# srv/pcl_feature_extraction

Hardware: AMD Instinct MI355X
Metric: Mpoints/s through NARF keypoint + FPFH descriptor on 1M-pt cloud (higher is better)
Workload: dtype f32; 1 GPU; configs[2] 1M-pt synthetic room, NARF(support 0.2) + normals(r 0.05) + FPFH(r 0.08) at the keypoints; image=640x480, parallelism=scan-per-gpu x1, descriptor_rows=83

## Files before the change

pcl_feature_extraction_amd/csrc/pfx_fpfh.hip:

```cpp
#include <cstring>
#include <rocprim/rocprim.hpp>

#include "pfx_nblist.h"
#include "pfx_neighbors.h"
#include "pfx_pair_features.h"

namespace pfx {
namespace {

constexpr int kBins = 11;
constexpr int kDesc = 33;
constexpr int kCapW = 8192;
constexpr int64_t kCapWGlobal = 1 << 22;
constexpr int kWOvfBlocks = 16;
constexpr int kChunkW = 128;
constexpr int kWT = 1024;
constexpr int kHistCopies = 16;


__device__ __forceinline__ bool bin_fast_nb(float v, float tol, int& h) {
  const float m = floorf(v);
  const float fr = v - m;
  h = (int)fminf(fmaxf(m, 0.0f), (float)(kBins - 1));
  return (fr > tol) & (fr < 1.0f - tol);
}

typedef float fv2 __attribute__((ext_vector_type(2)));
struct v32 { fv2 x, y, z; };
__device__ __forceinline__ fv2 dot4v(const v32& a, const v32& b) { return (a.x * b.x + a.z * b.z) + (a.y * b.y + 0.0f); }
__device__ __forceinline__ v32 cross3v(const v32& a, const v32& b) {
  return v32{a.y * b.z - a.z * b.y, a.z * b.x - a.x * b.z, a.x * b.y - a.y * b.x};
}
__device__ __forceinline__ fv2 sel2(bool c0, bool c1, fv2 a, fv2 b) { return fv2{c0 ? a.x : b.x, c1 ? a.y : b.y}; }

__device__ __forceinline__ void pair_bins_fast2(f3 p1, f3 n1, bool n1fin, const v32& p2, const v32& n2, int h1[2],
                                                int h2[2], int h3[2], bool ok[2]) {
  const int bz1 = bin_of<kBins>(f1_scaled<kBins>(0.0)), bz = bin_of<kBins>((double)kBins * ((0.0 + 1.0) * 0.5));
  const v32 dp0{p2.x - p1.x, p2.y - p1.y, p2.z - p1.z};
  const fv2 s4 = (dp0.x * dp0.x + dp0.z * dp0.z) + (dp0.y * dp0.y + 0.0f);
  const v32 n1v{fv2(n1.x), fv2(n1.y), fv2(n1.z)};
  const fv2 d1 = dot4v(n1v, dp0), d2 = dot4v(n2, dp0);
  bool sw[2], live[2];
  fv2 rf4;
#pragma unroll
  for (int c = 0; c < 2; ++c) {
    const bool fin = n1fin && isfinite(n2.x[c]) && isfinite(n2.y[c]) && isfinite(n2.z[c]);
    const float ad1 = fabsf(d1[c]), ad2 = fabsf(d2[c]);
    rf4[c] = __builtin_amdgcn_rsqf(s4[c]);
    sw[c] = ad1 < ad2 * (1.0f - 4e-7f);
    const bool decided = sw[c] || ad1 > ad2 * (1.0f + 4e-7f);
    live[c] = fin && !(fmaxf(ad1, ad2) * rf4[c] < 2e-8f) && decided;
  }
  const fv2 f3a = sel2(sw[0], sw[1], -d2 * rf4, d1 * rf4);
  const v32 n1c{sel2(sw[0], sw[1], n2.x, n1v.x), sel2(sw[0], sw[1], n2.y, n1v.y), sel2(sw[0], sw[1], n2.z, n1v.z)};
  const v32 n2c{sel2(sw[0], sw[1], n1v.x, n2.x), sel2(sw[0], sw[1], n1v.y, n2.y), sel2(sw[0], sw[1], n1v.z, n2.z)};
  const v32 dp{sel2(sw[0], sw[1], -dp0.x, dp0.x), sel2(sw[0], sw[1], -dp0.y, dp0.y), sel2(sw[0], sw[1], -dp0.z, dp0.z)};
  const v32 v = cross3v(dp, n1c);
  const fv2 sv = (v.x * v.x + v.z * v.z) + (v.y * v.y + 0.0f);
  const fv2 rsv{__builtin_amdgcn_rsqf(sv.x), __builtin_amdgcn_rsqf(sv.y)};
  const v32 vh{v.x * rsv, v.y * rsv, v.z * rsv};
  const v32 w = cross3v(n1c, vh);
  const fv2 f2a = dot4v(vh, n2c), y = dot4v(w, n2c), x = dot4v(n1c, n2c);
  fv2 mn, rmx;
  bool big[2];
#pragma unroll
  for (int c = 0; c < 2; ++c) {
    const float ax = fabsf(x[c]), ay = fabsf(y[c]);
    const float mx = fmaxf(ax, ay);
    mn[c] = fminf(ax, ay);
    big[c] = mx > 1e-20f;
    rmx[c] = __builtin_amdgcn_rcpf(mx);
  }
  const fv2 a = mn * rmx;
  const fv2 z = a * a;
  fv2 pp = fv2(-0.00405456405133009f);
  pp = pp * z + 0.021862948313355446f;
  pp = pp * z + -0.0559123195707798f;
  pp = pp * z + 0.0964219719171524f;
  pp = pp * z + -0.1390862911939621f;
  pp = pp * z + 0.19946566224098206f;
  pp = pp * z + -0.33329859375953674f;
  pp = pp * z + 0.9999993443489075f;
  fv2 t = pp * a;
#pragma unroll
  for (int c = 0; c < 2; ++c) {
    float tc = t[c];
    if (fabsf(y[c]) > fabsf(x[c])) tc = 1.57079637f - tc;
    if (x[c] < 0.0f) tc = 3.14159274f - tc;
    t[c] = y[c] < 0.0f ? -tc : tc;
  }
  const float d_pi = 1.0f / (2.0f * 3.14159265358979323846f);
  const fv2 tol1 = (fv2(1e-6f) + 8e-6f * rmx) * (1.01f * (float)kBins * d_pi) + kBinMapSlack;
  const fv2 b1 = (t + 3.14159265358979323846f) * ((float)kBins * d_pi);
  const fv2 b2 = (f2a + 1.0f) * (0.5f * kBins), b3 = (f3a + 1.0f) * (0.5f * kBins);
#pragma unroll
  for (int c = 0; c < 2; ++c) {
    int a1, a2, a3;
    const bool k1 = bin_fast_nb(b1[c], tol1[c], a1);
    const bool k2 = bin_fast_nb(b2[c], 4e-6f * 0.5f * kBins + kBinMapSlack, a2);
    const bool k3 = bin_fast_nb(b3[c], 1e-6f * 0.5f * kBins + kBinMapSlack, a3);
    const bool zero = s4[c] == 0.0f;
    ok[c] = zero | (live[c] & big[c] & k1 & k2 & k3);
    h1[c] = zero ? bz1 : a1;
    h2[c] = zero ? bz : a2;
    h3[c] = zero ? bz : a3;
  }
}

__device__ __attribute__((noinline)) int pair_bins_exact(float p1x, float p1y, float p1z, float n1x, float n1y,
                                                         float n1z, float p2x, float p2y, float p2z, float n2x,
                                                         float n2y, float n2z) {
  int h1, h2, h3;
  pair_bins<kBins>(mk3(p1x, p1y, p1z), mk3(n1x, n1y, n1z), mk3(p2x, p2y, p2z), mk3(n2x, n2y, n2z), h1, h2, h3);
  return h1 | (h2 << 8) | (h3 << 16);
}

__global__ void k_sorted_normals(const int32_t* __restrict__ perm, int64_t n, const float* __restrict__ nx,
                                 const float* __restrict__ ny, const float* __restrict__ nz,
                                 const uint8_t* __restrict__ support, float4* __restrict__ out,
                                 int* __restrict__ zero9) {
  const int64_t i = blockIdx.x * (int64_t)blockDim.x + threadIdx.x;
  if (zero9 && i < 9) zero9[i] = 0;
  if (i >= n) return;
  const int32_t p = perm[i];
  if (support && !support[p]) {
    out[i] = make_float4(__builtin_nanf(""), __builtin_nanf(""), __builtin_nanf(""), 0.0f);
    return;
  }
  out[i] = make_float4(nx[p], ny[p], nz[p], 0.0f);
}

__global__ void __launch_bounds__(256) k_fpfh_mark(GridView g, const float* __restrict__ qx,
                                                   const float* __restrict__ qy, const float* __restrict__ qz,
                                                   int64_t nq, float rr, uint8_t* __restrict__ flags) {
  for (int64_t q = blockIdx.x; q < nq; q += gridDim.x) {
    Runs R;
    const float x = qx[q], y = qy[q], z = qz[q];
    query_runs(g, x, y, z, R);
    for (int32_t t = threadIdx.x; t < R.pref[9]; t += blockDim.x) {
      const int32_t p = run_pos(R, t);
      const float4 c = g.sp[p];
      if (flann_d2(x, y, z, c.x, c.y, c.z) < rr) flags[p] = 1;
    }
  }
}

__global__ void __launch_bounds__(256) k_fpfh_mark_support(GridView g, const int32_t* __restrict__ plist,
                                                           const int64_t* __restrict__ n_ptr, float rr,
                                                           uint8_t* __restrict__ mask) {
  const int64_t n = *n_ptr;
  for (int64_t w = blockIdx.x; w < n; w += gridDim.x) {
    Runs R;
    const float4 q = g.sp[plist[w]];
    query_runs(g, q.x, q.y, q.z, R);
    for (int32_t t = threadIdx.x; t < R.pref[9]; t += blockDim.x) {
      const int32_t p = run_pos(R, t);
      const float4 c = g.sp[p];
      if (flann_d2(q.x, q.y, q.z, c.x, c.y, c.z) < rr) mask[g.perm[p]] = 1;
    }
  }
}

__global__ void __launch_bounds__(256) k_fpfh_mark_ball(GridView g, const float* __restrict__ qx,
                                                        const float* __restrict__ qy, const float* __restrict__ qz,
                                                        int64_t nq, float rr4, uint8_t* __restrict__ mask) {
  for (int64_t q = blockIdx.x; q < nq; q += gridDim.x) {
    const float x = qx[q], y = qy[q], z = qz[q];
    if (!(isfinite(x) && isfinite(y) && isfinite(z))) continue;
    const int64_t cx = (int64_t)floor(((double)x - g.ox) * g.inv);
    const int64_t cy = (int64_t)floor(((double)y - g.oy) * g.inv);
    const int64_t cz = (int64_t)floor(((double)z - g.oz) * g.inv);
    const int64_t z0 = max<int64_t>(cz - 2, 0), z1 = min<int64_t>(cz + 2, g.nz - 1);
    if (z0 > z1) continue;
    for (int c = 0; c < 25; ++c) {
      const int64_t ix = cx + c / 5 - 2, iy = cy + c % 5 - 2;
      if (ix < 0 || ix >= g.nx || iy < 0 || iy >= g.ny) continue;
      const int64_t base = (ix * g.ny + iy) * g.nz;
      const int32_t p0 = g.cell_start[base + z0], p1 = g.cell_start[base + z1 + 1];
      for (int32_t p = p0 + threadIdx.x; p < p1; p += blockDim.x) {
        const float4 c4 = g.sp[p];
        if (flann_d2(x, y, z, c4.x, c4.y, c4.z) <= rr4) mask[g.perm[p]] = 1;
      }
    }
  }
}

__global__ void k_all_finite(const uint32_t* __restrict__ skeys, int64_t n, uint64_t ncells,
                             uint8_t* __restrict__ flags) {
  const int64_t i = blockIdx.x * (int64_t)blockDim.x + threadIdx.x;
  if (i < n) flags[i] = (uint64_t)skeys[i] < ncells;
}

#ifndef PFX_SPFH_WPE
#define PFX_SPFH_WPE 7
#endif
__global__ void __launch_bounds__(256, PFX_SPFH_WPE) k_fpfh_spfh(GridView g, const float4* __restrict__ snp,
                                                      const int32_t* __restrict__ slist,
                                                      const int64_t* __restrict__ count_ptr, float rr,
                                                      int* __restrict__ hcount, int* __restrict__ kcount,
                                                      int2* __restrict__ slowq, unsigned* __restrict__ n_slow,
                                                      unsigned slow_cap, unsigned long long* __restrict__ pairs) {
  __shared__ uint32_t queue[4][192];
  __shared__ int hist[4][kHistCopies][kDesc];
  const int lane = threadIdx.x & 63, wv = __builtin_amdgcn_readfirstlane(threadIdx.x >> 6);
  const int64_t count = *count_ptr;
  const int64_t stride = (int64_t)gridDim.x * 4;
  unsigned long long wpairs = 0;
  for (int64_t w = xcd_block(blockIdx.x, gridDim.x) * 4 + wv; w < count; w += stride) {
    const int32_t s = __builtin_amdgcn_readfirstlane(slist[w]);
    float4 pc = g.sp[s], pnc = snp[s];
    pc.x = uniformf(pc.x); pc.y = uniformf(pc.y); pc.z = uniformf(pc.z);
    pnc.x = uniformf(pnc.x); pnc.y = uniformf(pnc.y); pnc.z = uniformf(pnc.z);
// ... 67 lines not shown
      for (int32_t t0 = 0; t0 < rn; t0 += 64) {
        const int32_t t = t0 + lane;
        bool hit = false;
        const int32_t pos = rs + t;
        if (t < rn) {
          const float4 c = g.sp[pos];
          hit = flann_d2(pc.x, pc.y, pc.z, c.x, c.y, c.z) < rr;
        }
        k += __popcll(__ballot(hit));
        const bool push = hit && pos != s;
        const uint64_t m = __ballot(push);
        if (push) queue[wv][qn + __popcll(m & lanemask_lt())] = (uint32_t)pos;
        qn += __popcll(m);
        if (qn >= 128) {
          process(128);
          const uint32_t rest = (lane + 128 < qn) ? queue[wv][lane + 128] : 0u;
          __builtin_amdgcn_fence(__ATOMIC_SEQ_CST, "wavefront");
          __builtin_amdgcn_wave_barrier();
          if (lane + 128 < qn) queue[wv][lane] = rest;
          qn -= 128;
        }
      }
    }
    process(qn);
    if (lane < kDesc) {
      int c = 0;
      for (int j = 0; j < kHistCopies; ++j) c += hist[wv][j][lane];
      hcount[w * kDesc + lane] = c;
    }
    if (lane == 0) kcount[w] = k;
    wpairs += (unsigned long long)(k - 1);
    __builtin_amdgcn_fence(__ATOMIC_SEQ_CST, "wavefront");
    __builtin_amdgcn_wave_barrier();
  }
  if (lane == 0 && wpairs) atomicAdd(pairs, wpairs);
}

__global__ void __launch_bounds__(256) k_fpfh_exact(GridView g, const float4* __restrict__ snp,
                                                    const int32_t* __restrict__ slist,
                                                    const int2* __restrict__ slowq, const unsigned* __restrict__ n_slow,
                                                    unsigned slow_cap, int* __restrict__ hcount,
                                                    unsigned long long* __restrict__ pairs) {
  const unsigned n = min(*n_slow, slow_cap);
  const unsigned i = blockIdx.x * 256 + threadIdx.x;
  if (i == 0) atomicAdd(pairs + 1, (unsigned long long)n);
  for (unsigned j = i; j < n; j += gridDim.x * 256) {
    const int2 e = slowq[j];
    const int32_t s = slist[e.x];
    const float4 pc = g.sp[s], pnc = snp[s], qc = g.sp[e.y], qnv = snp[e.y];
    const int hb = pair_bins_exact(pc.x, pc.y, pc.z, pnc.x, pnc.y, pnc.z, qc.x, qc.y, qc.z, qnv.x, qnv.y, qnv.z);
    int* hc = hcount + (int64_t)e.x * kDesc;
    atomicAdd(&hc[hb & 0xff], 1);
    atomicAdd(&hc[kBins + ((hb >> 8) & 0xff)], 1);
    atomicAdd(&hc[2 * kBins + (hb >> 16)], 1);
  }
}

__global__ void __launch_bounds__(256) k_fpfh_finalize(GridView g, const int32_t* __restrict__ slist,
                                                       const int64_t* __restrict__ count_ptr,
                                                       const int* __restrict__ hcount,
                                                       const int* __restrict__ kcount, float* __restrict__ spfh) {
  const int64_t count = *count_ptr;
  for (int64_t e = (int64_t)blockIdx.x * 256 + threadIdx.x; e < count * kDesc; e += (int64_t)gridDim.x * 256) {
    const int64_t w = e / kDesc;
    const int b = (int)(e - w * kDesc);
    const float incr = 100.0f / (float)(kcount[w] - 1);
    spfh[(int64_t)g.perm[slist[w]] * kDesc + b] = repeated_add(incr, hcount[e]);
  }
}

__device__ __forceinline__ int lsb_exp(float v) {
  const uint32_t b = __float_as_uint(v);
  const int e = (int)((b >> 23) & 0xff);
  if (e == 255) return 1000;
  const uint32_t m = (b & 0x7fffffu) | (e ? 0x800000u : 0u);
  return (e ? e : 1) - 150 + __builtin_ctz(m);
}

__device__ __forceinline__ int lsb_exp_bound(float v) {
  const int e = (int)((__float_as_uint(v) >> 23) & 0xff);
  return e == 255 ? 1000 : (e ? e : 1) - 150;
}

template <bool GLOBAL>
__global__ void __launch_bounds__(kWT) k_fpfh_weight(GridView g, const float* __restrict__ qx,
                                                     const float* __restrict__ qy, const float* __restrict__ qz,
                                                     int64_t nq, float rr, const float* __restrict__ spfh,
                                                     float* __restrict__ out, int* __restrict__ err,
                                                     int32_t* __restrict__ ovf, int* __restrict__ n_ovf,
                                                     uint64_t* __restrict__ scratch, int gcap) {
  extern __shared__ __attribute__((aligned(16))) uint64_t keys_lds[];
  __shared__ BucketLdsT<kWT> SB;
  uint64_t* keys = GLOBAL ? scratch + (size_t)blockIdx.x * gcap : keys_lds;
  const int kcap = GLOBAL ? gcap : kCapW;
  __shared__ float rows[kChunkW][kDesc + 1];
  __shared__ float wts[kChunkW];
  __shared__ double red_s[3][kWT / 64];
  __shared__ int red_l[3][kWT / 64];
  __shared__ int s_count;
  __shared__ double s_sum[3];
  const int tid = threadIdx.x;
  const int64_t count = GLOBAL ? (int64_t)*n_ovf : nq;
  for (int64_t w = blockIdx.x; w < count; w += gridDim.x) {
    const int64_t q = GLOBAL ? (int64_t)ovf[w] : w;
    const int k = GLOBAL ? sorted_neighbors(g, qx[q], qy[q], qz[q], rr, keys, kcap, &s_count)
                         : sorted_neighbors_bucketed<kWT>(g, qx[q], qy[q], qz[q], rr, keys, keys + kCapW, kcap,
                                                          &s_count, SB);
    if (k > kcap) {
      const bool give_up = GLOBAL || !ovf;
      if (tid == 0) {
        if (give_up) atomicMax(err, k);
        else ovf[atomicAdd(n_ovf, 1)] = (int32_t)q;
      }
      if (give_up && tid < kDesc) out[q * kDesc + tid] = __builtin_nanf("");
      continue;
    }
    if (k == 0) {
      if (tid < kDesc) out[q * kDesc + tid] = __builtin_nanf("");
      __syncthreads();
      continue;
    }
    float fh = 0.0f;
    double ps0 = 0.0, ps1 = 0.0, ps2 = 0.0;
    int pl0 = 1 << 20, pl1 = 1 << 20, pl2 = 1 << 20;
    constexpr int RS = kDesc + 1;
    float* rb0 = GLOBAL ? &rows[0][0] : reinterpret_cast<float*>(keys_lds + kCapW);
    float* rb1 = GLOBAL ? rb0 : rb0 + kChunkW * RS;
    const int nch = (k + kChunkW - 1) / kChunkW;
    auto stage = [&](int c, float* rbuf, int t0, int nt) {
      const int c0 = c * kChunkW, m = min(kChunkW, k - c0), tot = m * kDesc;
      constexpr int PER = (kChunkW * kDesc + (kWT - 64) - 1) / (kWT - 64);
      float v[PER];
#pragma unroll
      for (int u = 0; u < PER; ++u) {
        const int e = min(t0 + u * nt, tot - 1);
        const int j = e / kDesc, b = e - j * kDesc;
        v[u] = spfh[(int64_t)key_idx(keys[c0 + j]) * kDesc + b];
      }
#pragma unroll
      for (int u = 0; u < PER; ++u) {
        const int e = t0 + u * nt;
        if (e < tot) {
          const int j = e / kDesc, b = e - j * kDesc;
          rbuf[j * RS + b] = v[u];
        }
      }
      for (int j = t0; j < m; j += nt) {
        const float d2 = key_d2(keys[c0 + j]);
        rbuf[j * RS + kDesc] = d2 == 0.0f ? 0.0f : 1.0f / d2;
      }
    };
    stage(0, rb0, tid, kWT);
    __syncthreads();
    for (int c = 0; c < nch; ++c) {
      const int c0 = c * kChunkW, m = min(kChunkW, k - c0);
      const float* cur = (c & 1) ? rb1 : rb0;
      if (!GLOBAL && tid >= 64 && c + 1 < nch) stage(c + 1, (c & 1) ? rb0 : rb1, tid - 64, kWT - 64);
      if (tid < kDesc) {
#pragma unroll 8
        for (int j = 0; j < m; ++j) fh = fh + cur[j * RS + tid] * cur[j * RS + kDesc];
      }
      const int pt0 = GLOBAL ? tid : tid - 64, pnt = GLOBAL ? kWT : kWT - 64;
      if (pt0 >= 0) {
        for (int e = pt0; e < m * kDesc; e += pnt) {
          const int j = e / kDesc, b = e - j * kDesc;
          const float w = cur[j * RS + kDesc];
          if (w == 0.0f) continue;
          const float v = cur[j * RS + b] * w;
          if (v != 0.0f) {
            const int l = lsb_exp(v);
            if (b < kBins) { ps0 += (double)v; pl0 = min(pl0, l); }
            else if (b < 2 * kBins) { ps1 += (double)v; pl1 = min(pl1, l); }
            else { ps2 += (double)v; pl2 = min(pl2, l); }
          }
        }
      }
      __syncthreads();
      if (GLOBAL && c + 1 < nch) {
        stage(c + 1, rb0, tid, kWT);
        __syncthreads();
      }
    }
#pragma unroll
    for (int o = 32; o > 0; o >>= 1) {
      ps0 += __shfl_xor(ps0, o); ps1 += __shfl_xor(ps1, o); ps2 += __shfl_xor(ps2, o);
      pl0 = min(pl0, __shfl_xor(pl0, o)); pl1 = min(pl1, __shfl_xor(pl1, o)); pl2 = min(pl2, __shfl_xor(pl2, o));
    }
    if ((tid & 63) == 0) {
      const int wv = tid >> 6;
      red_s[0][wv] = ps0; red_s[1][wv] = ps1; red_s[2][wv] = ps2;
      red_l[0][wv] = pl0; red_l[1][wv] = pl1; red_l[2][wv] = pl2;
    }
    __syncthreads();
    if (tid < 3) {
      double t = 0.0;
      int l = 1 << 20;
      for (int wv = 0; wv < kWT / 64; ++wv) { t += red_s[tid][wv]; l = min(l, red_l[tid][wv]); }
      red_s[tid][0] = t;
      red_l[tid][0] = l;
    }
    __shared__ int s_inexact;
    if (tid == 0) {
      s_inexact = 0;
      atomicMax(err + 1, k);
    }
    __syncthreads();
    if (tid < 3) {
      const int blk = tid;
      const double sum = red_s[blk][0];
      const int L = red_l[blk][0];
      const bool exact = sum == 0.0 || (L < 1000 && sum < ldexp(1.0, L + 52));
      s_sum[blk] = sum;
      if (!exact) atomicOr(&s_inexact, 1 << blk);
    }
    __syncthreads();
    const int inexact = s_inexact;
    if (tid == 0 && inexact) atomicAdd(err + 2, 1);
    if (inexact) {
      double seq = 0.0;
      for (int c0 = 0; c0 < k; c0 += kChunkW) {
        const int m = min(kChunkW, k - c0);
        for (int e = tid; e < m * kDesc; e += kWT) {
          const int j = e / kDesc, b = e - j * kDesc;
          rows[j][b] = spfh[(int64_t)key_idx(keys[c0 + j]) * kDesc + b];
        }
        if (tid < m) {
          const float d2 = key_d2(keys[c0 + tid]);
          wts[tid] = d2 == 0.0f ? 0.0f : 1.0f / d2;
        }
        __syncthreads();
        if (tid < 3 && ((inexact >> tid) & 1)) {
          for (int j = 0; j < m; ++j) {
            const float w = wts[j];
            if (w == 0.0f) continue;
#pragma unroll
            for (int b = 0; b < kBins; ++b) seq = seq + (double)(rows[j][tid * kBins + b] * w);
          }
        }
        __syncthreads();
      }
      if (tid < 3 && ((inexact >> tid) & 1)) s_sum[tid] = seq;
      __syncthreads();
    }
    if (tid < 3) {
      double sum = s_sum[tid];
      if (sum != 0.0) sum = 100.0 / sum;
      s_sum[tid] = sum;
    }
    __syncthreads();
    if (tid < kDesc) out[q * kDesc + tid] = fh * (float)s_sum[tid / kBins];
    __syncthreads();
  }
}

#ifndef PFX_WL_PIPE
#define PFX_WL_PIPE 2
#endif
#ifndef PFX_W_BLOCKS
#define PFX_W_BLOCKS 512
#endif
#ifndef PFX_WL_GRID
#define PFX_WL_GRID 32
#endif
__device__ __forceinline__ int32_t entry_pos(uint32_t e, const int32_t (&rs)[9]) {
// ... 173 lines not shown
      }
      scale = sum != 0.0 ? 100.0 / sum : 0.0;
      s_ps[wv][lane] = scale;
    }
    __builtin_amdgcn_fence(__ATOMIC_SEQ_CST, "wavefront");
    __builtin_amdgcn_wave_barrier();
    if (lane < kDesc) out[(int64_t)qi * kDesc + lane] = fh * (float)s_ps[wv][lane / kBins];
    kmax = max(kmax, k);
    __builtin_amdgcn_fence(__ATOMIC_SEQ_CST, "wavefront");
    __builtin_amdgcn_wave_barrier();
  }
  if (lane == 0 && kmax) atomicMax(err + 1, kmax);
}

__global__ void k_nan_rows_nonfinite(const float* __restrict__ x, const float* __restrict__ y,
                                     const float* __restrict__ z, int64_t n, float* __restrict__ out) {
  const int64_t e = blockIdx.x * (int64_t)blockDim.x + threadIdx.x;
  if (e >= n * kDesc) return;
  const int64_t i = e / kDesc;
  if (!(isfinite(x[i]) && isfinite(y[i]) && isfinite(z[i]))) out[e] = __builtin_nanf("");
}

}

void fpfh_prepare_dev(pfx_ctx* ctx, const float* sx, const float* sy, const float* sz, int64_t ns, double r) {
  ctx->prep_x = nullptr;
  ctx->prep_n = -1;
  ctx->prep_qx = nullptr;
  ctx->prep_nq = -1;
  if (ns == 0) return;
  build_grid(ctx, ctx->grid_b, sx, sy, sz, ns, r, true);
  if (ctx->grid_b.oob) {
    if (!ctx->grid_b_hoob) PFX_HIP(hipHostMalloc((void**)&ctx->grid_b_hoob, 64, hipHostMallocDefault));
    if (!ctx->grid_b_oob_ev) PFX_HIP(hipEventCreateWithFlags(&ctx->grid_b_oob_ev, hipEventDisableTiming));
    PFX_HIP(hipMemcpyAsync(ctx->grid_b_hoob, ctx->grid_b.oob, sizeof(int), hipMemcpyDeviceToHost, ctx->stream));
    PFX_HIP(hipEventRecord(ctx->grid_b_oob_ev, ctx->stream));
  }
  ctx->prep_x = sx;
  ctx->prep_n = ns;
  ctx->prep_r = r;
}

bool fpfh_validate_grid(pfx_ctx* ctx) {
  Grid& G = ctx->grid_b;
  if (!G.oob) return false;
  G.oob = nullptr;
  PFX_HIP(hipEventSynchronize(ctx->grid_b_oob_ev));
  if (*ctx->grid_b_hoob == 0) return false;
  note_grid_word(ctx, G, *ctx->grid_b_hoob);
  ctx->stats["fpfh_speculative_reruns"] += 1;
  const float* x = ctx->prep_x;
  const int64_t n = ctx->prep_n;
  const double r = ctx->prep_r;
  build_grid(ctx, G, G.ux, G.uy, G.uz, G.n, r);
  ctx->prep_x = x;
  ctx->prep_n = n;
  ctx->prep_r = r;
  return true;
}

void fpfh_prepare_queries_dev(pfx_ctx* ctx, const float* sx, const float* sy, const float* sz, int64_t ns,
                              const float* qx, const float* qy, const float* qz, int64_t nq, double r) {
  PFX_CHECK(r > 0.0, "fpfh_prepare_queries: radius must be > 0");
  ctx->prep_qx = nullptr;
  ctx->prep_nq = -1;
  if (ns == 0 || nq == 0) return;
  if (!(ctx->prep_x == sx && ctx->prep_n == ns && ctx->prep_r == r)) fpfh_prepare_dev(ctx, sx, sy, sz, ns, r);
  fpfh_validate_grid(ctx);
  hipStream_t st = ctx->stream;
  const Grid& G = ctx->grid_b;
  uint8_t* flags = ctx->buf("fpfh_flags").as<uint8_t>(ns);
  int32_t* slist = ctx->buf("fpfh_list").as<int32_t>(ns);
  int64_t* d_sel = ctx->buf("fpfh_nsel").as<int64_t>(1);
  size_t tmp_bytes = 0;
  PFX_HIP(rocprim::select(nullptr, tmp_bytes, rocprim::counting_iterator<int32_t>(0), flags, slist, d_sel,
                          (size_t)ns, st));
  void* tmp = ctx->buf("fpfh_tmp").get(tmp_bytes + 16);
  TimeScope ts(ctx, "fpfh_prepare_queries");
  PFX_HIP(hipMemsetAsync(flags, 0, ns, st));
  k_fpfh_mark<<<(unsigned)std::min<int64_t>(nq, 8192), 256, 0, st>>>(view(G), qx, qy, qz, nq, (float)(r * r), flags);
  check_launch("k_fpfh_mark");
  PFX_HIP(rocprim::select(tmp, tmp_bytes, rocprim::counting_iterator<int32_t>(0), flags, slist, d_sel, (size_t)ns,
                          st));
  ctx->prep_qx = qx;
  ctx->prep_nq = nq;
}

void fpfh_support_mask_dev(pfx_ctx* ctx, const float* sx, const float* sy, const float* sz, int64_t ns,
                           const float* qx, const float* qy, const float* qz, int64_t nq, double r, uint8_t* mask) {
  PFX_CHECK(r > 0.0, "fpfh support: radius must be > 0");
  ctx->fpfh_support = nullptr;
  if (ns == 0) return;
  hipStream_t st = ctx->stream;
  PFX_HIP(hipMemsetAsync(mask, 0, ns, st));
  if (nq == 0) return;
  if (!(ctx->prep_x == sx && ctx->prep_n == ns && ctx->prep_r == r)) fpfh_prepare_dev(ctx, sx, sy, sz, ns, r);
  fpfh_validate_grid(ctx);
  TimeScope ts(ctx, "fpfh_support");
  const Grid& G = ctx->grid_b;
  const GridView g = view(G);
  const float rr = (float)(r * r);
  uint8_t* flags = ctx->buf("fpfh_sflags").as<uint8_t>(ns);
  int32_t* slist = ctx->buf("fpfh_slist").as<int32_t>(ns);
  int64_t* d_sel = ctx->buf("fpfh_snsel").as<int64_t>(1);
  size_t tmp_bytes = 0;
  PFX_HIP(rocprim::select(nullptr, tmp_bytes, rocprim::counting_iterator<int32_t>(0), flags, slist, d_sel,
                          (size_t)ns, st));
  void* tmp = ctx->buf("fpfh_stmp").get(tmp_bytes + 16);
  PFX_HIP(hipMemsetAsync(flags, 0, ns, st));
  k_fpfh_mark<<<(unsigned)std::min<int64_t>(nq, 8192), 256, 0, st>>>(g, qx, qy, qz, nq, rr, flags);
  PFX_HIP(rocprim::select(tmp, tmp_bytes, rocprim::counting_iterator<int32_t>(0), flags, slist, d_sel, (size_t)ns,
                          st));
  k_fpfh_mark_support<<<8192, 256, 0, st>>>(g, slist, d_sel, rr, mask);
  check_launch("k_fpfh_mark_support");
  ctx->fpfh_support = mask;
}

void fpfh_support_ball_dev(pfx_ctx* ctx, const float* sx, const float* sy, const float* sz, int64_t ns,
                           const float* qx, const float* qy, const float* qz, int64_t nq, double r, uint8_t* mask) {
  PFX_CHECK(r > 0.0, "fpfh support: radius must be > 0");
  ctx->fpfh_support = nullptr;
  if (ns == 0) return;
  hipStream_t st = ctx->stream;
  PFX_HIP(hipMemsetAsync(mask, 0, ns, st));
  if (nq == 0) return;
  if (!(ctx->prep_x == sx && ctx->prep_n == ns && ctx->prep_r == r)) fpfh_prepare_dev(ctx, sx, sy, sz, ns, r);
  fpfh_validate_grid(ctx);
  TimeScope ts(ctx, "fpfh_support");
  const float rr4 = (float)(4.0 * r * r * (1.0 + 1e-5));
  k_fpfh_mark_ball<<<(unsigned)std::min<int64_t>(nq, 8192), 256, 0, st>>>(view(ctx->grid_b), qx, qy, qz, nq, rr4,
                                                                          mask);
  check_launch("k_fpfh_mark_ball");
  ctx->fpfh_support = mask;
}

void fpfh_dev(pfx_ctx* ctx, const float* sx, const float* sy, const float* sz, const float* snx,
              const float* sny, const float* snz, int64_t ns, const float* qx, const float* qy, const float* qz,
              int64_t nq, int same, double r, float* out, bool reuse_normal_lists) {
  PFX_CHECK(r > 0.0, "fpfh: radius must be > 0");
  if (nq == 0) return;
  hipStream_t st = ctx->stream;
  if (ns == 0) {
    std::vector<float> nanrow((size_t)nq * kDesc, __builtin_nanf(""));
    PFX_HIP(hipMemcpyAsync(out, nanrow.data(), sizeof(float) * nanrow.size(), hipMemcpyHostToDevice, st));
    PFX_HIP(hipStreamSynchronize(st));
    return;
  }
  const bool grid_ready = ctx->prep_x == sx && ctx->prep_n == ns && ctx->prep_r == r;
  if (!grid_ready) build_grid(ctx, ctx->grid_b, sx, sy, sz, ns, r);
  const bool rebuilt = grid_ready && fpfh_validate_grid(ctx);
  const bool s_ready = grid_ready && !rebuilt && !same && ctx->prep_qx == qx && ctx->prep_nq == nq;
  ctx->prep_x = nullptr;
  ctx->prep_n = -1;
  ctx->prep_qx = nullptr;
  ctx->prep_nq = -1;
  const Grid& G = ctx->grid_b;
  GridView g = view(G);
  const float rr = (float)(r * r);
  float* spfh = ctx->buf("fpfh_spfh").as<float>(ns * kDesc);
  float4* snp = ctx->buf("fpfh_snp").as<float4>(ns);
  uint8_t* flags = ctx->buf("fpfh_flags").as<uint8_t>(ns);
  int32_t* slist = ctx->buf("fpfh_list").as<int32_t>(ns);
  int64_t* d_sel = ctx->buf("fpfh_nsel").as<int64_t>(1);
  size_t tmp_bytes = 0;
  PFX_HIP(rocprim::select(nullptr, tmp_bytes, rocprim::counting_iterator<int32_t>(0), flags, slist, d_sel,
                          (size_t)ns, st));
  void* tmp = ctx->buf("fpfh_tmp").get(tmp_bytes + 16);
  const unsigned nb = (unsigned)ceil_div(ns, 256);
  DevBuf& eb = ctx->buf("fpfh_err");
  const bool fresh = !eb.ptr;
  int* err = eb.as<int>(10);
  if (fresh) PFX_HIP(hipMemsetAsync(err, 0, 10 * sizeof(int), st));
  {
    TimeScope ts(ctx, "fpfh_mark");
    k_sorted_normals<<<nb, 256, 0, st>>>(G.perm, ns, snx, sny, snz, same ? nullptr : ctx->fpfh_support, snp,
                                         err + 1);
    ctx->fpfh_support = nullptr;
    if (!s_ready) {
      if (same) {
        k_all_finite<<<nb, 256, 0, st>>>(G.skeys, ns, (uint64_t)G.ncells, flags);
      } else {
        PFX_HIP(hipMemsetAsync(flags, 0, ns, st));
        k_fpfh_mark<<<(unsigned)std::min<int64_t>(nq, 8192), 256, 0, st>>>(g, qx, qy, qz, nq, rr, flags);
      }
      check_launch("k_fpfh_mark");
      PFX_HIP(rocprim::select(tmp, tmp_bytes, rocprim::counting_iterator<int32_t>(0), flags, slist, d_sel,
                              (size_t)ns, st));
    }
  }
  const bool overflow_pass = ns > kCapW;
  int32_t* ovf = overflow_pass ? ctx->buf("fpfh_wovf").as<int32_t>(nq) : nullptr;
  const int gcap = overflow_pass ? (int)std::min<int64_t>(kCapWGlobal, (int64_t)1 << (64 - __builtin_clzll((unsigned long long)ns - 1))) : 0;
  uint64_t* wscratch = overflow_pass ? ctx->buf("fpfh_wscratch").as<uint64_t>((size_t)kWOvfBlocks * gcap) : nullptr;
  unsigned long long* d_pairs = reinterpret_cast<unsigned long long*>(err + 4);
  unsigned* n_slow = reinterpret_cast<unsigned*>(err + 3);
  int* hcount = ctx->buf("fpfh_hcount").as<int>(ns * kDesc);
  int* kcount = ctx->buf("fpfh_kcount").as<int>(ns);
  const char* cap_env = getenv("PFX_FPFH_SLOW_CAP");
  const unsigned slow_cap = cap_env ? (unsigned)std::max(1, atoi(cap_env)) : 1u << 20;
  int2* slowq = ctx->buf("fpfh_slowq").as<int2>(slow_cap);
  {
    TimeScope ts(ctx, "fpfh_spfh", true);
    const int64_t waves = std::min<int64_t>(ns, 256 * 4 * 16);
    k_fpfh_spfh<<<(unsigned)std::max<int64_t>(8, ceil_div(waves, 4) & ~7), 256, 0, st>>>(
        g, snp, slist, d_sel, rr, hcount, kcount, slowq, n_slow, slow_cap, d_pairs);
    k_fpfh_exact<<<256, 256, 0, st>>>(g, snp, slist, slowq, n_slow, slow_cap, hcount, d_pairs);
    k_fpfh_finalize<<<(unsigned)std::min<int64_t>(ceil_div(ns * kDesc, 256), 4096), 256, 0, st>>>(
        g, slist, d_sel, hcount, kcount, spfh);
    check_launch("k_fpfh_spfh");
  }
  if (same) {
    TimeScope ts(ctx, "fpfh_weight", true);
    NormalsState* nst = ctx->normals;
    const bool reuse = reuse_normal_lists && nst && nst->ready && nst->x == sx && nst->y == sy && nst->z == sz &&
                       nst->n == ns && nst->r == r;
    if (nst && reuse_normal_lists) nst->ready = false;
    NbLists L;
    if (reuse) L = nst->L;
    else build_lists(ctx, G, nullptr, r, true, L, "fpfh");
    ctx->stats["fpfh_weight_lists_reused"] = reuse ? 1 : 0;
    k_nan_rows_nonfinite<<<(unsigned)ceil_div(ns * kDesc, 256), 256, 0, st>>>(sx, sy, sz, ns, out);
    if (L.nq > 0)
    {
      const unsigned bl = (unsigned)std::min<int64_t>(ceil_div(L.nq, 4), 256 * PFX_WL_GRID);
      const GridView gv = reuse ? view(ctx->grid_a) : g;
      const bool buf = ns * kDesc * 4 < ((int64_t)1 << 31);
      if (buf)
        k_fpfh_weight_lists<true><<<bl, 256, 0, st>>>(gv, L.qpos, L.off, L.cnt, L.lg, L.list, L.skeys, L.nq, spfh, out, err);
      else
        k_fpfh_weight_lists<false><<<bl, 256, 0, st>>>(gv, L.qpos, L.off, L.cnt, L.lg, L.list, L.skeys, L.nq, spfh, out,
                                                       err);
    }
    check_launch("k_fpfh_weight_lists");
  } else {
    TimeScope ts(ctx, "fpfh_weight", true);
    const size_t lds = sizeof(uint64_t) * 2 * kCapW;
    PFX_HIP(hipFuncSetAttribute((const void*)k_fpfh_weight<false>, hipFuncAttributeMaxDynamicSharedMemorySize, (int)lds));
    const unsigned blocks = (unsigned)std::min<int64_t>(nq, PFX_W_BLOCKS);
    k_fpfh_weight<false><<<blocks, kWT, lds, st>>>(g, qx, qy, qz, nq, rr, spfh, out, err, ovf, err + 8, nullptr, 0);
    if (overflow_pass)
      k_fpfh_weight<true><<<kWOvfBlocks, kWT, 0, st>>>(g, qx, qy, qz, nq, rr, spfh, out, err, ovf, err + 8, wscratch,
                                                        gcap);
    check_launch("k_fpfh_weight");
  }
  FpfhReadback* rb = ctx->fpfh_rb();
  PFX_HIP(hipMemcpyAsync(rb->h, err, sizeof(rb->h), hipMemcpyDeviceToHost, st));
  PFX_HIP(hipMemcpyAsync(&rb->count, d_sel, sizeof(int64_t), hipMemcpyDeviceToHost, st));
  rb->slow_cap = slow_cap;
  ctx->fpfh_pending = true;
}

void fpfh_resolve(pfx_ctx* ctx) {
  if (!ctx->fpfh_pending) return;
  ctx->fpfh_pending = false;
  const FpfhReadback* rb = ctx->fpfh_rb();
  const int* h = rb->h;
  const unsigned n_slow = (unsigned)h[3];
  ctx->stats["fpfh_spfh_points"] = rb->count;
  unsigned long long pr;
  std::memcpy(&pr, h + 4, sizeof(pr));
  ctx->stats["fpfh_spfh_pairs"] = (int64_t)pr;
  std::memcpy(&pr, h + 6, sizeof(pr));
  ctx->stats["fpfh_spfh_exact_pairs"] = (int64_t)pr;
  ctx->stats["fpfh_spfh_deferred"] = n_slow;
  ctx->stats["fpfh_spfh_inline_exact"] = n_slow > rb->slow_cap ? n_slow - rb->slow_cap : 0;
  ctx->stats["fpfh_weight_kmax"] = h[1];
  ctx->stats["fpfh_weight_sequential"] = h[2];
  ctx->stats["fpfh_weight_global"] = h[8];
  if (h[0] > 0) {
    int* err = ctx->buf("fpfh_err").as<int>(10);
    PFX_HIP(hipMemsetAsync(err, 0, sizeof(int), ctx->stream));
    throw Error(PFX_ERR_CAPACITY, "fpfh: a query has " + std::to_string(h[0]) + " neighbours (> " +
                                      std::to_string(kCapWGlobal) + " supported)");
  }
}

}
```

pcl_feature_extraction_amd/csrc/pfx_internal.h:

```cpp
#pragma once
#include <hip/hip_runtime.h>
#include <stdint.h>
#include <cstdlib>

#include <map>
#include <stdexcept>
#include <string>
#include <vector>

#include "../../include/pfx.h"

namespace pfx {

struct Error : std::runtime_error {
  pfx_status code;
  Error(pfx_status c, const std::string& m) : std::runtime_error(m), code(c) {}
};

#define PFX_HIP(expr)                                                                   \
  do {                                                                                  \
    hipError_t _e = (expr);                                                             \
    if (_e != hipSuccess)                                                               \
      throw ::pfx::Error(PFX_ERR_DEVICE, std::string(#expr) + ": " + hipGetErrorString(_e)); \
  } while (0)
// ... 32 lines not shown
    PFX_HIP(hipEventCreate(&e));
    return e;
  }
};

struct Grid {
  int64_t n = 0;
  float cell = 0.f, inv = 0.f, ox = 0.f, oy = 0.f, oz = 0.f;
  double dinv = 0.0, dox = 0.0, doy = 0.0, doz = 0.0;
  int32_t nx = 0, ny = 0, nz = 0;
  int64_t ncells = 0;
  float *sx = nullptr, *sy = nullptr, *sz = nullptr;
  float4* sp = nullptr;
  const float *ux = nullptr, *uy = nullptr, *uz = nullptr;
  int32_t* perm = nullptr;
  int32_t* cell_start = nullptr;
  const uint32_t* skeys = nullptr;
  DevBuf b_sx, b_sy, b_sz, b_sp, b_perm, b_start, b_keys, b_keys2, b_vals, b_tmp, b_minmax, b_oob, b_scr, b_fat;
  bool have_hint = false;
  double hint_lo[3] = {0, 0, 0}, hint_hi[3] = {0, 0, 0};
  int* oob = nullptr;
  mutable bool fat = false;
  int* h_fat = nullptr;
  hipEvent_t fat_ev = nullptr;
  bool fat_pending = false;
  bool hint_user = false;
  bool counted = false;
  uint64_t gen = 0;
  void release() {
    b_sx.release(); b_sy.release(); b_sz.release(); b_sp.release(); b_perm.release(); b_start.release();
    b_keys.release(); b_keys2.release(); b_vals.release(); b_tmp.release(); b_minmax.release(); b_oob.release();
    b_scr.release(); b_fat.release();
    if (fat_ev) { (void)hipEventSynchronize(fat_ev); (void)hipEventDestroy(fat_ev); fat_ev = nullptr; }
    if (h_fat) { (void)hipHostFree(h_fat); h_fat = nullptr; }
    fat_pending = false;
    have_hint = false;
    fat = false;
    oob = nullptr;
    ++gen;
  }
};

constexpr int kGridFatCap = 1024;
constexpr int kGridFatBit = 1 << 30;

struct GridView {
  const float *sx, *sy, *sz;
  const float4* sp;
  const float *ux, *uy, *uz;
  const int32_t* perm;
  const int32_t* cell_start;
  double inv, ox, oy, oz;
  int32_t nx, ny, nz;
};

struct FpfhReadback {
  int h[10];
  int64_t count;
  unsigned slow_cap;
};

struct NarfState;
struct NormalsState;
struct KeypointState;
struct IcpState;

}

struct pfx_ctx {
  int device = 0;
  hipStream_t own_stream = nullptr;
  hipStream_t stream = nullptr;
  bool on_own_stream = true;
  std::string last_error;
  bool shared_device = false;
  pfx::KernelTimer timer;
  std::map<std::string, int64_t> stats;
  pfx::Grid grid_a, grid_b;
  const float* prep_x = nullptr;
  int64_t prep_n = -1;
  double prep_r = 0.0;
  const float* prep_qx = nullptr;
  int64_t prep_nq = -1;
  const uint8_t* fpfh_support = nullptr;
  int* grid_b_hoob = nullptr;
  hipEvent_t grid_b_oob_ev = nullptr;
  std::map<std::string, pfx::DevBuf> bufs;
  pfx::NarfState* narf = nullptr;
  pfx::NormalsState* normals = nullptr;
  hipEvent_t lists_gate = nullptr;
  bool normals_fork_hint = true;
  pfx::KeypointState* kp = nullptr;
  pfx::IcpState* icp = nullptr;
  pfx::DevBuf& buf(const char* name) { return bufs[name]; }
  void* fpfh_rb_mem = nullptr;
  bool fpfh_pending = false;
  pfx::FpfhReadback* fpfh_rb() {
    if (!fpfh_rb_mem) PFX_HIP(hipHostMalloc(&fpfh_rb_mem, sizeof(pfx::FpfhReadback), hipHostMallocDefault));
    return static_cast<pfx::FpfhReadback*>(fpfh_rb_mem);
  }
  void* pfh_rb_mem = nullptr;
  bool pfh_pending = false;
  void* spin_rb_mem = nullptr;
  bool spin_pending = false;
  void* rift_rb_mem = nullptr;
  bool igrad_pending = false, rift_pending = false;
  hipStream_t side = nullptr;
  hipEvent_t fork_ev[2] = {nullptr, nullptr};
  hipEvent_t spin_ev = nullptr;
  void sync_spin(hipStream_t st) {
    if (!spin_ev) PFX_HIP(hipEventCreateWithFlags(&spin_ev, hipEventDisableTiming));
    PFX_HIP(hipEventRecord(spin_ev, st));
    hipError_t e;
    while ((e = hipEventQuery(spin_ev)) == hipErrorNotReady) {
    }
    PFX_HIP(e);
  }
  void ensure_side() {
    if (side) return;
    int prio = 0;
    if (stream) PFX_HIP(hipStreamGetPriority(stream, &prio));
    PFX_HIP(hipStreamCreateWithPriority(&side, hipStreamNonBlocking, prio));
    for (auto& e : fork_ev) PFX_HIP(hipEventCreateWithFlags(&e, hipEventDisableTiming));
  }
  void* host_rb = nullptr;
  template <class T> T* readback() {
    if (!host_rb) PFX_HIP(hipHostMalloc(&host_rb, 4096, hipHostMallocDefault));
    return static_cast<T*>(host_rb);
  }
  void* host_scratch = nullptr;
  size_t host_scratch_bytes = 0;
  void* pinned(size_t need) {
    if (need > host_scratch_bytes) {
      if (host_scratch) {
        PFX_HIP(hipStreamSynchronize(stream));
        PFX_HIP(hipHostFree(host_scratch));
      }
      host_scratch_bytes = need + need / 2 + 4096;
      PFX_HIP(hipHostMalloc(&host_scratch, host_scratch_bytes, hipHostMallocDefault));
    }
    return host_scratch;
  }
};

namespace pfx {

struct TimeScope {
  pfx_ctx* ctx;
  hipEvent_t a = nullptr, b = nullptr;
  std::string name;
  TimeScope(pfx_ctx* c, std::string n, bool stage = false) : ctx(c), name(std::move(n)) {
    if (ctx->timer.enabled && (stage || !ctx->timer.stages_only)) {
      a = ctx->timer.take();
      b = ctx->timer.take();
      PFX_HIP(hipEventRecord(a, ctx->stream));
    }
  }
  ~TimeScope() {
    if (a) {
      (void)hipEventRecord(b, ctx->stream);
      ctx->timer.pending.push_back(KernelTimer::Pending{a, b, name});
    }
  }
};

inline void check_launch(const char* what) {
// ... 126 lines not shown
```

Before: 212.9 Mpoints/s.

## Precompute FPFH neighbor keys in prep pass and deepen weight-stage pipeline

When the query count is small, a new prep kernel computes each keypoint's sorted radius neighbor keys once and stores them in global memory. The prepared-keys weight kernel loads those keys instead of redoing the bucketed neighbor search. It also uses larger chunks with register-prefetched loads one chunk ahead and a per-column partial-sum layout. Sorted normals are now gathered only for grid cells near the queries rather than for the whole cloud. The cost is extra global scratch of nq*8192 keys, more LDS per block, and added code paths gated on the query count.

```diff
diff --git a/pcl_feature_extraction_amd/csrc/pfx_fpfh.hip b/pcl_feature_extraction_amd/csrc/pfx_fpfh.hip
--- a/pcl_feature_extraction_amd/csrc/pfx_fpfh.hip
+++ b/pcl_feature_extraction_amd/csrc/pfx_fpfh.hip
@@ -14,6 +14,9 @@
 constexpr int64_t kCapWGlobal = 1 << 22;
 constexpr int kWOvfBlocks = 16;
 constexpr int kChunkW = 128;
+constexpr int kStageDepth = 2;
+constexpr int kChunkP = kStageDepth * kChunkW;
+constexpr int64_t kPrepMaxQ = 512;
 constexpr int kWT = 1024;
 constexpr int kHistCopies = 16;
 
@@ -128,6 +131,36 @@
     return;
   }
   out[i] = make_float4(nx[p], ny[p], nz[p], 0.0f);
+}
+
+__global__ void __launch_bounds__(256) k_sorted_normals_ball(GridView g, const float* __restrict__ qx,
+                                                             const float* __restrict__ qy,
+                                                             const float* __restrict__ qz, int64_t nq,
+                                                             const float* __restrict__ nx, const float* __restrict__ ny,
+                                                             const float* __restrict__ nz,
+                                                             const uint8_t* __restrict__ support,
+                                                             float4* __restrict__ out, int* __restrict__ zero9) {
+  if (zero9 && blockIdx.x == 0 && threadIdx.x < 9) zero9[threadIdx.x] = 0;
+  for (int64_t w = blockIdx.x; w < nq * 25; w += gridDim.x) {
+    const int64_t q = w / 25;
+    const int c = (int)(w - q * 25);
+    const float x = qx[q], y = qy[q], z = qz[q];
+    if (!(isfinite(x) && isfinite(y) && isfinite(z))) continue;
+    const int64_t cx = (int64_t)floor(((double)x - g.ox) * g.inv);
+    const int64_t cy = (int64_t)floor(((double)y - g.oy) * g.inv);
+    const int64_t cz = (int64_t)floor(((double)z - g.oz) * g.inv);
+    const int64_t z0 = max<int64_t>(cz - 2, 0), z1 = min<int64_t>(cz + 2, g.nz - 1);
+    const int64_t ix = cx + c / 5 - 2, iy = cy + c % 5 - 2;
+    if (z0 > z1 || ix < 0 || ix >= g.nx || iy < 0 || iy >= g.ny) continue;
+    const int64_t base = (ix * g.ny + iy) * g.nz;
+    const int32_t p0 = g.cell_start[base + z0], p1 = g.cell_start[base + z1 + 1];
+    for (int32_t i = p0 + threadIdx.x; i < p1; i += 256) {
+      const int32_t p = g.perm[i];
+      const bool in = !support || support[p];
+      const float nan = __builtin_nanf("");
+      out[i] = in ? make_float4(nx[p], ny[p], nz[p], 0.0f) : make_float4(nan, nan, nan, 0.0f);
+    }
+  }
 }
 
 __global__ void __launch_bounds__(256) k_fpfh_mark(GridView g, const float* __restrict__ qx,
@@ -361,17 +394,39 @@
   return e == 255 ? 1000 : (e ? e : 1) - 150;
 }
 
-template <bool GLOBAL>
+__global__ void __launch_bounds__(kWT) k_fpfh_prep_keys(GridView g, const float* __restrict__ qx,
+                                                        const float* __restrict__ qy, const float* __restrict__ qz,
+                                                        int64_t nq, float rr, uint64_t* __restrict__ pkeys,
+                                                        int* __restrict__ pcount) {
+  extern __shared__ __attribute__((aligned(16))) uint64_t keys_lds[];
+  __shared__ BucketLdsT<kWT> SB;
+  __shared__ int s_count;
+  const int tid = threadIdx.x;
+  for (int64_t q = blockIdx.x; q < nq; q += gridDim.x) {
+    const int k = sorted_neighbors_bucketed<kWT>(g, qx[q], qy[q], qz[q], rr, keys_lds, keys_lds + kCapW, kCapW,
+                                                 &s_count, SB);
+    if (tid == 0) pcount[q] = k;
+    if (k <= kCapW)
+      for (int i = tid; i < k; i += kWT) pkeys[q * kCapW + i] = keys_lds[i];
+    __syncthreads();
+  }
+}
+
+template <bool GLOBAL, bool PREP = false>
 __global__ void __launch_bounds__(kWT) k_fpfh_weight(GridView g, const float* __restrict__ qx,
                                                      const float* __restrict__ qy, const float* __restrict__ qz,
                                                      int64_t nq, float rr, const float* __restrict__ spfh,
                                                      float* __restrict__ out, int* __restrict__ err,
                                                      int32_t* __restrict__ ovf, int* __restrict__ n_ovf,
-                                                     uint64_t* __restrict__ scratch, int gcap) {
+                                                     uint64_t* __restrict__ scratch, int gcap,
+                                                     const uint64_t* __restrict__ pkeys,
+                                                     const int* __restrict__ pcount) {
+  static_assert(!(GLOBAL && PREP), "prepared keys are the LDS pass's");
   extern __shared__ __attribute__((aligned(16))) uint64_t keys_lds[];
   __shared__ BucketLdsT<kWT> SB;
   uint64_t* keys = GLOBAL ? scratch + (size_t)blockIdx.x * gcap : keys_lds;
   const int kcap = GLOBAL ? gcap : kCapW;
+  constexpr int CH = PREP ? kChunkP : kChunkW;
   __shared__ float rows[kChunkW][kDesc + 1];
   __shared__ float wts[kChunkW];
   __shared__ double red_s[3][kWT / 64];
@@ -382,9 +437,24 @@
   const int64_t count = GLOBAL ? (int64_t)*n_ovf : nq;
   for (int64_t w = blockIdx.x; w < count; w += gridDim.x) {
     const int64_t q = GLOBAL ? (int64_t)ovf[w] : w;
-    const int k = GLOBAL ? sorted_neighbors(g, qx[q], qy[q], qz[q], rr, keys, kcap, &s_count)
-                         : sorted_neighbors_bucketed<kWT>(g, qx[q], qy[q], qz[q], rr, keys, keys + kCapW, kcap,
-                                                          &s_count, SB);
+    int k;
+    if constexpr (PREP) {
+      k = pcount[q];
+      if (k <= kCapW) {
+        const uint64_t* pk = pkeys + q * kCapW;
+        uint64_t kv[kCapW / kWT];
+#pragma unroll
+        for (int u = 0; u < kCapW / kWT; ++u) kv[u] = pk[max(min(tid + u * kWT, k - 1), 0)];
+#pragma unroll
+        for (int u = 0; u < kCapW / kWT; ++u)
+          if (tid + u * kWT < k) keys[tid + u * kWT] = kv[u];
+        __syncthreads();
+      }
+    } else if constexpr (GLOBAL) {
+      k = sorted_neighbors(g, qx[q], qy[q], qz[q], rr, keys, kcap, &s_count);
+    } else {
+      k = sorted_neighbors_bucketed<kWT>(g, qx[q], qy[q], qz[q], rr, keys, keys + kCapW, kcap, &s_count, SB);
+    }
     if (k > kcap) {
       const bool give_up = GLOBAL || !ovf;
       if (tid == 0) {
@@ -404,18 +474,20 @@
     int pl0 = 1 << 20, pl1 = 1 << 20, pl2 = 1 << 20;
     constexpr int RS = kDesc + 1;
     float* rb0 = GLOBAL ? &rows[0][0] : reinterpret_cast<float*>(keys_lds + kCapW);
-    float* rb1 = GLOBAL ? rb0 : rb0 + kChunkW * RS;
-    const int nch = (k + kChunkW - 1) / kChunkW;
-    auto stage = [&](int c, float* rbuf, int t0, int nt) {
-      const int c0 = c * kChunkW, m = min(kChunkW, k - c0), tot = m * kDesc;
-      constexpr int PER = (kChunkW * kDesc + (kWT - 64) - 1) / (kWT - 64);
-      float v[PER];
+    float* rb1 = GLOBAL ? rb0 : rb0 + CH * RS;
+    const int nch = (k + CH - 1) / CH;
+    constexpr int PER = (CH * kDesc + (kWT - 64) - 1) / (kWT - 64);
+    auto load = [&](int c, int t0, int nt, float (&v)[PER]) {
+      const int c0 = c * CH, tot = min(CH, k - c0) * kDesc;
 #pragma unroll
       for (int u = 0; u < PER; ++u) {
         const int e = min(t0 + u * nt, tot - 1);
         const int j = e / kDesc, b = e - j * kDesc;
         v[u] = spfh[(int64_t)key_idx(keys[c0 + j]) * kDesc + b];
       }
+    };
+    auto store = [&](int c, float* rbuf, int t0, int nt, const float (&v)[PER]) {
+      const int c0 = c * CH, m = min(CH, k - c0), tot = m * kDesc;
 #pragma unroll
       for (int u = 0; u < PER; ++u) {
         const int e = t0 + u * nt;
@@ -429,18 +501,66 @@
         rbuf[j * RS + kDesc] = d2 == 0.0f ? 0.0f : 1.0f / d2;
       }
     };
+    auto stage = [&](int c, float* rbuf, int t0, int nt) {
+      float v[PER];
+      load(c, t0, nt, v);
+      store(c, rbuf, t0, nt, v);
+    };
     stage(0, rb0, tid, kWT);
+    constexpr int NR = (kWT - 64) / kDesc, PERF = (CH + NR - 1) / NR;
+    const int ft = tid - 64;
+    const bool fon = PREP && ft >= 0 && ft < NR * kDesc;
+    const int fr = fon ? ft / kDesc : 0, fb = fon ? ft - fr * kDesc : 0;
+    auto loadf = [&](int c, float (&v)[PERF]) {
+      const int c0 = c * CH, m = min(CH, k - c0);
+#pragma unroll
+      for (int u = 0; u < PERF; ++u) v[u] = spfh[(int64_t)key_idx(keys[c0 + min(fr + u * NR, m - 1)]) * kDesc + fb];
+    };
+    auto storef = [&](int c, float* rbuf, const float (&v)[PERF]) {
+      const int c0 = c * CH, m = min(CH, k - c0);
+      if (fon) {
+#pragma unroll
+        for (int u = 0; u < PERF; ++u)
+          if (fr + u * NR < m) rbuf[(fr + u * NR) * RS + fb] = v[u];
+      }
+      for (int j = ft; j < m; j += kWT - 64) {
+        const float d2 = key_d2(keys[c0 + j]);
+        rbuf[j * RS + kDesc] = d2 == 0.0f ? 0.0f : 1.0f / d2;
+      }
+    };
+    float pv[PERF];
+    double fps = 0.0;
+    int fpl = 1 << 20;
+    if constexpr (PREP) {
+      if (tid >= 64 && nch > 1) loadf(1, pv);
+    }
     __syncthreads();
     for (int c = 0; c < nch; ++c) {
-      const int c0 = c * kChunkW, m = min(kChunkW, k - c0);
+      const int c0 = c * CH, m = min(CH, k - c0);
       const float* cur = (c & 1) ? rb1 : rb0;
-      if (!GLOBAL && tid >= 64 && c + 1 < nch) stage(c + 1, (c & 1) ? rb0 : rb1, tid - 64, kWT - 64);
+      if constexpr (PREP) {
+        if (tid >= 64 && c + 1 < nch) {
+          storef(c + 1, (c & 1) ? rb0 : rb1, pv);
+          if (c + 2 < nch) loadf(c + 2, pv);
+        }
+      } else if (!GLOBAL && tid >= 64 && c + 1 < nch) {
+        stage(c + 1, (c & 1) ? rb0 : rb1, tid - 64, kWT - 64);
+      }
       if (tid < kDesc) {
 #pragma unroll 8
         for (int j = 0; j < m; ++j) fh = fh + cur[j * RS + tid] * cur[j * RS + kDesc];
       }
       const int pt0 = GLOBAL ? tid : tid - 64, pnt = GLOBAL ? kWT : kWT - 64;
-      if (pt0 >= 0) {
+      if constexpr (PREP) {
+        if (fon) {
+          for (int j = fr; j < m; j += NR) {
+            const float w = cur[j * RS + kDesc];
+            const float v = w == 0.0f ? 0.0f : cur[j * RS + fb] * w;
+            fps += (double)v;
+            fpl = v != 0.0f ? min(fpl, lsb_exp(v)) : fpl;
+          }
+        }
+      } else if (pt0 >= 0) {
         for (int e = pt0; e < m * kDesc; e += pnt) {
           const int j = e / kDesc, b = e - j * kDesc;
           const float w = cur[j * RS + kDesc];
@@ -459,6 +579,11 @@
         stage(c + 1, rb0, tid, kWT);
         __syncthreads();
       }
+    }
+    if (fon) {
+      if (fb < kBins) { ps0 = fps; pl0 = fpl; }
+      else if (fb < 2 * kBins) { ps1 = fps; pl1 = fpl; }
+      else { ps2 = fps; pl2 = fpl; }
     }
 #pragma unroll
     for (int o = 32; o > 0; o >>= 1) {
@@ -798,6 +923,15 @@
   check_launch("k_fpfh_mark");
   PFX_HIP(rocprim::select(tmp, tmp_bytes, rocprim::counting_iterator<int32_t>(0), flags, slist, d_sel, (size_t)ns,
                           st));
+  ctx->prep_keys = nq <= kPrepMaxQ;
+  if (ctx->prep_keys) {
+    uint64_t* pkeys = ctx->buf("fpfh_pkeys").as<uint64_t>((size_t)nq * kCapW);
+    int* pcount = ctx->buf("fpfh_pcount").as<int>(nq);
+    const size_t lds = sizeof(uint64_t) * 2 * kCapW;
+    PFX_HIP(hipFuncSetAttribute((const void*)k_fpfh_prep_keys, hipFuncAttributeMaxDynamicSharedMemorySize, (int)lds));
+    k_fpfh_prep_keys<<<(unsigned)nq, kWT, lds, st>>>(view(G), qx, qy, qz, nq, (float)(r * r), pkeys, pcount);
+    check_launch("k_fpfh_prep_keys");
+  }
   ctx->prep_qx = qx;
   ctx->prep_nq = nq;
 }
@@ -866,10 +1000,12 @@
   if (!grid_ready) build_grid(ctx, ctx->grid_b, sx, sy, sz, ns, r);
   const bool rebuilt = grid_ready && fpfh_validate_grid(ctx);
   const bool s_ready = grid_ready && !rebuilt && !same && ctx->prep_qx == qx && ctx->prep_nq == nq;
+  const bool k_ready = s_ready && ctx->prep_keys;
   ctx->prep_x = nullptr;
   ctx->prep_n = -1;
   ctx->prep_qx = nullptr;
   ctx->prep_nq = -1;
+  ctx->prep_keys = false;
   const Grid& G = ctx->grid_b;
   GridView g = view(G);
   const float rr = (float)(r * r);
@@ -889,8 +1025,12 @@
   if (fresh) PFX_HIP(hipMemsetAsync(err, 0, 10 * sizeof(int), st));
   {
     TimeScope ts(ctx, "fpfh_mark");
-    k_sorted_normals<<<nb, 256, 0, st>>>(G.perm, ns, snx, sny, snz, same ? nullptr : ctx->fpfh_support, snp,
-                                         err + 1);
+    if (!same && nq * 4096 <= ns)
+      k_sorted_normals_ball<<<(unsigned)(nq * 25), 256, 0, st>>>(g, qx, qy, qz, nq, snx, sny, snz, ctx->fpfh_support,
+                                                                 snp, err + 1);
+    else
+      k_sorted_normals<<<nb, 256, 0, st>>>(G.perm, ns, snx, sny, snz, same ? nullptr : ctx->fpfh_support, snp,
+                                           err + 1);
     ctx->fpfh_support = nullptr;
     if (!s_ready) {
       if (same) {
@@ -950,13 +1090,25 @@
     check_launch("k_fpfh_weight_lists");
   } else {
     TimeScope ts(ctx, "fpfh_weight", true);
-    const size_t lds = sizeof(uint64_t) * 2 * kCapW;
-    PFX_HIP(hipFuncSetAttribute((const void*)k_fpfh_weight<false>, hipFuncAttributeMaxDynamicSharedMemorySize, (int)lds));
     const unsigned blocks = (unsigned)std::min<int64_t>(nq, PFX_W_BLOCKS);
-    k_fpfh_weight<false><<<blocks, kWT, lds, st>>>(g, qx, qy, qz, nq, rr, spfh, out, err, ovf, err + 8, nullptr, 0);
+    ctx->stats["fpfh_weight_prepared"] = k_ready ? 1 : 0;
+    if (k_ready) {
+      const size_t lds = sizeof(uint64_t) * kCapW + sizeof(float) * 2 * kChunkP * (kDesc + 1);
+      PFX_HIP(hipFuncSetAttribute((const void*)k_fpfh_weight<false, true>, hipFuncAttributeMaxDynamicSharedMemorySize,
+                                  (int)lds));
+      k_fpfh_weight<false, true><<<blocks, kWT, lds, st>>>(g, qx, qy, qz, nq, rr, spfh, out, err, ovf, err + 8, nullptr,
+                                                           0, ctx->buf("fpfh_pkeys").as<uint64_t>((size_t)nq * kCapW),
+                                                           ctx->buf("fpfh_pcount").as<int>(nq));
+    } else {
+      const size_t lds = sizeof(uint64_t) * 2 * kCapW;
+      PFX_HIP(hipFuncSetAttribute((const void*)k_fpfh_weight<false>, hipFuncAttributeMaxDynamicSharedMemorySize,
+                                  (int)lds));
+      k_fpfh_weight<false><<<blocks, kWT, lds, st>>>(g, qx, qy, qz, nq, rr, spfh, out, err, ovf, err + 8, nullptr, 0,
+                                                     nullptr, nullptr);
+    }
     if (overflow_pass)
       k_fpfh_weight<true><<<kWOvfBlocks, kWT, 0, st>>>(g, qx, qy, qz, nq, rr, spfh, out, err, ovf, err + 8, wscratch,
-                                                        gcap);
+                                                        gcap, nullptr, nullptr);
     check_launch("k_fpfh_weight");
   }
   FpfhReadback* rb = ctx->fpfh_rb();
diff --git a/pcl_feature_extraction_amd/csrc/pfx_internal.h b/pcl_feature_extraction_amd/csrc/pfx_internal.h
--- a/pcl_feature_extraction_amd/csrc/pfx_internal.h
+++ b/pcl_feature_extraction_amd/csrc/pfx_internal.h
@@ -138,6 +138,7 @@
   double prep_r = 0.0;
   const float* prep_qx = nullptr;
   int64_t prep_nq = -1;
+  bool prep_keys = false;
   const uint8_t* fpfh_support = nullptr;
   int* grid_b_hoob = nullptr;
   hipEvent_t grid_b_oob_ev = nullptr;
```

New measurement: 215.9 Mpoints/s, median of 6. 1.01x the previous value.
